# alibaba/euler

Measured on NVIDIA H100. Metric: sampled_edges_per_sec, higher is better.
Workload: dtype u64 ids / f32 weights+features (f64 CDF compare)

## Files before the change

euler_b200/csrc/internal.h:

```cpp
#pragma once
#include <cuda_runtime.h>
#include <stdint.h>

#include <string.h>

#include <atomic>
#include <string>
#include <type_traits>
#include <vector>

#include "../../include/euler_b200.h"
#include "common.cuh"

namespace eu {

void set_error(const char* fmt, ...);
extern std::atomic<uint64_t> g_launches;

#define EU_CUDA(call)                                                                    \
  do {                                                                                   \
    cudaError_t _e = (call);                                                             \
    if (_e != cudaSuccess) {                                                             \
      ::eu::set_error("%s:%d %s -> %s", __FILE__, __LINE__, #call, cudaGetErrorString(_e)); \
      return EU_ERR_CUDA;                                                                \
// ... 68 lines not shown
  float type_fwc_sum = 0.f;
  float* d_type_prob = nullptr;
  int32_t* d_type_alias = nullptr;
  std::vector<int64_t> sampler_order;
  std::vector<std::string> edge_type_names, node_type_names;
  std::vector<std::string> dense_feature_names;
  std::vector<std::string> sparse_feature_names, binary_feature_names;
  std::vector<uint64_t> u64_slot_max;
  eu::DevEdges e{};
  bool edges_set = false;
  struct EdgeSampler { int64_t n = 0; const int64_t* order = nullptr; const float* prob = nullptr; const int32_t* alias = nullptr; float fwc_sum = 0.f; };
  std::vector<EdgeSampler> edge_samplers;
  std::vector<std::string> edge_dense_names, edge_sparse_names, edge_binary_names;
  bool labels_built = false;
  std::vector<std::string> labels;
  int32_t* d_label_ptr = nullptr;
  unsigned long long* d_label_ids = nullptr;

  template <typename T>
  int alloc(T** p, int64_t count) {
    size_t bytes = (size_t)(count > 0 ? count : 1) * sizeof(T);
    bytes = (bytes + 255) & ~(size_t)255;
    void* q = nullptr;
    cudaError_t e = cudaMalloc(&q, bytes);
    if (e != cudaSuccess) {
      eu::set_error("cudaMalloc(%zu) -> %s", bytes, cudaGetErrorString(e));
      return EU_ERR_CUDA;
    }
    allocs.push_back(q);
    hbm_bytes += (int64_t)bytes;
    *p = (T*)q;
    return EU_OK;
  }
  template <typename T>
  int host_alloc(T** host, T** dev, int64_t count) {
    const size_t bytes = (size_t)(count > 0 ? count : 1) * sizeof(T);
    void* q = nullptr;
    cudaError_t e = cudaHostAlloc(&q, bytes, cudaHostAllocMapped);
    if (e != cudaSuccess) {
      cudaGetLastError();
      eu::set_error("cudaHostAlloc(%zu, mapped) -> %s", bytes, cudaGetErrorString(e));
      return EU_ERR_CUDA;
    }
    host_allocs.push_back(q);
    host_bytes += (int64_t)bytes;
    void* qd = nullptr;
    e = cudaHostGetDevicePointer(&qd, q, 0);
    if (e != cudaSuccess) { eu::set_error("cudaHostGetDevicePointer -> %s", cudaGetErrorString(e)); return EU_ERR_CUDA; }
    *host = (T*)q;
    *dev = (T*)qd;
    return EU_OK;
  }
};

struct EuRngState {
  uint32_t x;
  uint32_t x_prev;
  unsigned long long draws;
  unsigned long long calls;
  unsigned int blocks_done;
  unsigned int pad2;
  unsigned long long key;
};

struct eu_ctx {
  eu_graph* g = nullptr;
  eu_rng_kind rng = EU_RNG_MINSTD;
  uint64_t seed = 0;
  cudaStream_t stream = nullptr;
  EuRngState* d_rng = nullptr;
  int n_eng = 1;
  int64_t cap_rows = 0;
  eu::HashSlot* d_dedup = nullptr;
  int64_t tab_set_slots = 0;
  int32_t* d_first = nullptr;
  int64_t* d_rowof = nullptr;
  uint8_t* d_elig = nullptr;
  uint32_t* d_state = nullptr;
  uint32_t* d_emask = nullptr;
  uint32_t* d_woff = nullptr;
  uint32_t* d_blkpre = nullptr;
  uint32_t* d_blkmul = nullptr;
  int32_t* d_live = nullptr;
  int32_t* d_dup = nullptr;
  unsigned int* d_nlive = nullptr;
  unsigned long long* d_front[2] = {nullptr, nullptr};
  int64_t agg_rows = 0, agg_slots = 0;
  unsigned long long* d_agg_tab = nullptr;
  int32_t* d_agg_src = nullptr;
  int32_t* d_agg_rep = nullptr;
  uint32_t* d_agg_slot = nullptr;
  unsigned int* d_agg_nrep = nullptr;
  void* d_misc = nullptr;
  int64_t misc_bytes = 0;
  float* d_walkv = nullptr;
  long long walkv_cap = 0;
  cudaStream_t aux[2] = {nullptr, nullptr};
  cudaEvent_t ev_fork = nullptr, ev_join[2] = {nullptr, nullptr};
  void* h_pin = nullptr;
  int64_t pin_bytes = 0;
  void* d_stage = nullptr;
  int64_t stage_bytes = 0;
  bool prof = false;
  struct ProfRec { const char* name; int64_t rows; cudaEvent_t e0, e1; };
  std::vector<ProfRec> prof_recs;
};

struct EuProfScope {
  eu_ctx* c; size_t idx;
  EuProfScope(eu_ctx* c_, const char* name, int64_t rows) : c(c_), idx((size_t)-1) {
    if (!c->prof) return;
    eu_ctx::ProfRec r{name, rows, nullptr, nullptr};
    cudaEventCreate(&r.e0); cudaEventCreate(&r.e1);
    cudaEventRecord(r.e0, c->stream);
    c->prof_recs.push_back(r);
    idx = c->prof_recs.size() - 1;
  }
  ~EuProfScope() { if (idx != (size_t)-1) cudaEventRecord(c->prof_recs[idx].e1, c->stream); }
};

namespace eu {
static constexpr int64_t kRepeatMinRows = (int64_t)1 << 17;
int ctx_reserve(eu_ctx* c, int64_t rows, int64_t table_slots);
int64_t hop_scratch_rows(int nb, int64_t rows_b);
int64_t hop_table_slots(int nb, int64_t rows_b);
int64_t hop_table_cap(int64_t rows_b);
int ctx_misc(eu_ctx* c, int64_t bytes);
inline size_t a256(size_t b) { return (b + 255) & ~(size_t)255; }
struct EdgeOrder;
int segmented_row_sum(eu_ctx* c, const float* rows, const float* w, const EdgeOrder& o, const int32_t* row, int64_t E, int64_t n,
                      int dim, float* out);
size_t ragged_scan_bytes(int64_t M);
int sparse_entry_ptr(eu_ctx* c, const int64_t* nodes, int64_t M, int32_t fid, void* tmp, size_t tmp_bytes, int64_t* ptr);
int agg_reserve(eu_ctx* c, int64_t rows, int64_t table_slots);
int refuse_growth_in_capture(eu_ctx* c, const char* what);
int graph_build_sampler(eu_graph* g);
int feat_storage_check(const eu_feat_storage* in, int64_t n, const char* who, eu_feat_storage* st);
int graph_build_labels(eu_graph* g);
void graph_label_list(const std::vector<int64_t>& order, int64_t n, const int64_t* bin_ptr, const uint8_t* bin_val, int32_t S,
                      int32_t fid, std::vector<std::string>* labels, std::vector<int32_t>* row_label);
__global__ void k_advance_engine(EuRngState* rng, unsigned long long uniforms);
__global__ void k_ragged_stats(const long long* __restrict__ ptr, int64_t rows, long long* __restrict__ stats);
int agnn_dot(eu_ctx* c, const float* a, const float* b, const int32_t* ia, const int32_t* ib, int64_t E, int dim,
             const float* beta, float* dot, float* scaled);
int get_node_weight(eu_ctx* c, const int64_t* nodes, int64_t B, float* out);
int launch_state_scan(eu_ctx* c, int64_t rows, unsigned long long uniforms_per_row);
int hop(eu_ctx* c, const unsigned long long* seeds, int64_t rows, const int32_t* etypes, int32_t K,
        int32_t count, int64_t default_node, unsigned long long* eng_ids, int64_t* out_ids,
        float* out_w, int32_t* out_t, int hop_index, bool pre_inserted, bool insert_next, int nb,
        const int32_t* rows_act = nullptr, bool raw = false);
}
```

euler_b200/csrc/mp_ops.cu:

```cuda
#include <stdlib.h>

#include <cooperative_groups.h>

#include <algorithm>

#include "segment.cuh"

namespace cg = cooperative_groups;

namespace eu {

__device__ __forceinline__ float4 ldg4(const float* p) { return __ldg(reinterpret_cast<const float4*>(p)); }
__device__ __forceinline__ void st4(float* p, float4 v) { *reinterpret_cast<float4*>(p) = v; }

template <typename T, bool VEC, int P>
__global__ void __launch_bounds__(256) k_feature(DevGraph g, const unsigned long long* __restrict__ ids,
                                                 int64_t M, int32_t dim, int G, int32_t soff, int32_t sdim,
                                                 float* __restrict__ out) {
  const int sh = 31 - __clz(G);
  const int sub = (int)(threadIdx.x & (G - 1));
  const int64_t stride = ((int64_t)gridDim.x * blockDim.x) >> sh;
  for (int64_t i = (blockIdx.x * (int64_t)blockDim.x + threadIdx.x) >> sh; i < M; i += stride) {
    const int64_t row = sdim > 0 ? lookup_row(g, ids[i]) : -1;
    const int32_t fd = sdim;
    float* o = out + i * (int64_t)dim;
    const T* f = row >= 0 ? feat_row<T, P>(g, row) + soff : nullptr;
    if (VEC) {
      for (int32_t d = sub * 4; d < dim; d += G * 4) {
        float4 v = make_float4(0.f, 0.f, 0.f, 0.f);
        if (f && d < fd) v = feat_ld4(f + d);
        st4(o + d, v);
      }
    } else {
      for (int32_t d = sub; d < dim; d += G) o[d] = (f && d < fd) ? feat_ld(f + d) : 0.f;
    }
  }
}

template <bool VEC>
__global__ void __launch_bounds__(256) k_gather(const float* __restrict__ params, int64_t D,
                                                const int32_t* __restrict__ idx, int64_t E, int G,
                                                float* __restrict__ out) {
  const int64_t tid = blockIdx.x * (int64_t)blockDim.x + threadIdx.x;
  const int64_t i = tid >> (31 - __clz(G));
  const int sub = (int)(tid & (G - 1));
  if (i >= E) return;
  const float* src = params + (int64_t)__ldg(idx + i) * D;
  float* o = out + i * D;
  if (VEC) {
    for (int64_t d = sub * 4; d < D; d += G * 4) st4(o + d, ldg4(src + d));
  } else {
    for (int64_t d = sub; d < D; d += G) o[d] = __ldg(src + d);
  }
}

enum { OP_ADD = 0, OP_MAX = 1, OP_MEAN = 2 };

template <int OP, bool VEC>
__global__ void __launch_bounds__(256) k_scatter_sorted(const float* __restrict__ upd, int64_t D,
                                                        const int32_t* __restrict__ idx, int64_t E,
                                                        int64_t size, int G, const int* unsorted,
                                                        float* __restrict__ out) {
  if (*unsorted) return;
  const int64_t tid = blockIdx.x * (int64_t)blockDim.x + threadIdx.x;
  const int64_t r = tid >> (31 - __clz(G));
  const int sub = (int)(tid & (G - 1));
  if (r >= size) return;
  const int64_t b = key_lower_bound(idx, E, r), e = key_lower_bound(idx, E, r + 1);
  const float init = OP == OP_MAX ? -1e9f : 0.f;
  const float denom = __fadd_rn((float)(e - b), 1e-7f);
  float* o = out + r * D;
  if (VEC) {
    for (int64_t d = sub * 4; d < D; d += G * 4) {
      float4 acc = make_float4(init, init, init, init);
      for (int64_t k = b; k < e; ++k) {
        float4 v = ldg4(upd + k * D + d);
        if (OP == OP_MAX) {
          acc.x = v.x > acc.x ? v.x : acc.x; acc.y = v.y > acc.y ? v.y : acc.y;
          acc.z = v.z > acc.z ? v.z : acc.z; acc.w = v.w > acc.w ? v.w : acc.w;
        } else {
          acc.x = __fadd_rn(acc.x, v.x); acc.y = __fadd_rn(acc.y, v.y);
          acc.z = __fadd_rn(acc.z, v.z); acc.w = __fadd_rn(acc.w, v.w);
        }
      }
      if (OP == OP_MEAN) {
        acc.x = __fdiv_rn(acc.x, denom); acc.y = __fdiv_rn(acc.y, denom);
        acc.z = __fdiv_rn(acc.z, denom); acc.w = __fdiv_rn(acc.w, denom);
      }
      st4(o + d, acc);
    }
  } else {
    for (int64_t d = sub; d < D; d += G) {
      float acc = init;
      for (int64_t k = b; k < e; ++k) {
        float v = __ldg(upd + k * D + d);
        if (OP == OP_MAX) acc = v > acc ? v : acc; else acc = __fadd_rn(acc, v);
      }
      if (OP == OP_MEAN) acc = __fdiv_rn(acc, denom);
      o[d] = acc;
    }
  }
}

__global__ void k_fill_if(float* __restrict__ out, int64_t n, float v, const int* unsorted) {
  if (!*unsorted) return;
  int64_t i = blockIdx.x * (int64_t)blockDim.x + threadIdx.x;
  const int64_t stride = (int64_t)gridDim.x * blockDim.x;
  for (; i < n; i += stride) out[i] = v;
}

__device__ __forceinline__ void atomic_max_f32(float* addr, float v) {
  if (v != v) return;
  if (__float_as_int(v) >= 0) atomicMax(reinterpret_cast<int*>(addr), __float_as_int(v));
  else atomicMin(reinterpret_cast<unsigned int*>(addr), __float_as_uint(v));
}

template <int OP, bool VEC>
__global__ void __launch_bounds__(256) k_scatter_atomic(const float* __restrict__ upd, int64_t D,
                                                        const int32_t* __restrict__ idx, int64_t E, int G,
                                                        const int* unsorted, float* __restrict__ out,
                                                        float* __restrict__ cnt) {
  if (!*unsorted) return;
  const int64_t tid = blockIdx.x * (int64_t)blockDim.x + threadIdx.x;
  const int64_t i = tid >> (31 - __clz(G));
  const int sub = (int)(tid & (G - 1));
  if (i >= E) return;
  const int64_t r = __ldg(idx + i);
  float* o = out + r * D;
  const float* u = upd + i * D;
  if (OP == OP_MEAN && sub == 0) atomicAdd(cnt + r, 1.0f);
  if (VEC && OP != OP_MAX) {
    for (int64_t d = sub * 4; d < D; d += G * 4) atomicAdd(reinterpret_cast<float4*>(o + d), ldg4(u + d));
  } else {
    const int step = VEC ? 4 : 1;
    for (int64_t d = sub * step; d < D; d += G * step)
      for (int q = 0; q < step; ++q) {
        if (OP == OP_MAX) atomic_max_f32(o + d + q, __ldg(u + d + q));
        else atomicAdd(o + d + q, __ldg(u + d + q));
      }
  }
}

__global__ void k_mean_div(float* __restrict__ out, int64_t D, int64_t size, const float* __restrict__ cnt,
                           const int* unsorted) {
  if (!*unsorted) return;
  int64_t i = blockIdx.x * (int64_t)blockDim.x + threadIdx.x;
  if (i < size * D) out[i] = __fdiv_rn(out[i], __fadd_rn(cnt[i / D], 1e-7f));
}

__global__ void __launch_bounds__(256) k_sage_classify(DevGraph g, const unsigned long long* __restrict__ ids, int64_t rows,
                                                       int32_t count, unsigned long long* tab, unsigned long long mask,
                                                       int32_t* __restrict__ src, int32_t* __restrict__ reps,
                                                       uint32_t* __restrict__ rep_slot, unsigned int* n_rep) {
  const int64_t stride = (int64_t)gridDim.x * blockDim.x;
  for (int64_t r = blockIdx.x * (int64_t)blockDim.x + threadIdx.x; r < rows; r += stride) {
    const unsigned long long* seg = ids + r * count;
    unsigned long long h = 0;
    bool any = false;
#pragma unroll 4
    for (int32_t j = 0; j < count; ++j) {
      const unsigned long long id = __ldg(seg + j);
      any |= lookup_row(g, id) >= 0;
      h = mix64(h + id + 1);
    }
    if (!any) { src[r] = -1; continue; }
    const unsigned long long tag = h & 0xFFFFFFFF00000000ull;
    unsigned long long p = h & mask;
    while (true) {
      unsigned long long sl = *reinterpret_cast<volatile unsigned long long*>(tab + p);
      if (sl == 0ull) {
        sl = atomicCAS(tab + p, 0ull, tag | (unsigned long long)(r + 1));
        if (sl == 0ull) {
          src[r] = (int32_t)r;
          const cg::coalesced_group grp = cg::coalesced_threads();
          unsigned int q = 0;
          if (grp.thread_rank() == 0) q = atomicAdd(n_rep, grp.size());
          q = grp.shfl(q, 0) + grp.thread_rank();
          reps[q] = (int32_t)r;
          rep_slot[q] = (uint32_t)p;
          break;
        }
      }
      if ((sl & 0xFFFFFFFF00000000ull) == tag) {
        const int64_t o = (int64_t)(sl & 0xFFFFFFFFull) - 1;
        const unsigned long long* os = ids + o * count;
        bool same = true;
#pragma unroll 4
        for (int32_t j = 0; j < count; ++j) same &= __ldg(seg + j) == __ldg(os + j);
        if (same) { src[r] = (int32_t)o; break; }
      }
      p = (p + 1) & mask;
    }
  }
}

template <typename T, int NV, bool FULL, int P>
__global__ void __launch_bounds__(256) k_sage_mean(DevGraph g, const unsigned long long* __restrict__ ids,
                                                   int64_t rows, const int32_t* __restrict__ list, const unsigned int* __restrict__ n_list,
                                                   int32_t count, bool mean, float* __restrict__ out) {
  const int lane = threadIdx.x & 31;
  const int32_t fd = FULL ? NV * 128 : g.feat_dim;
  const int64_t nwarps = ((int64_t)gridDim.x * blockDim.x) >> 5;
  const int64_t n = list ? (int64_t)__ldg(n_list) : rows;
  for (int64_t q = (blockIdx.x * (int64_t)blockDim.x + threadIdx.x) >> 5; q < n; q += nwarps) {
  const int64_t r = list ? (int64_t)__ldg(list + q) : q;
  float4 acc[NV];
#pragma unroll
  for (int v = 0; v < NV; ++v) acc[v] = make_float4(0.f, 0.f, 0.f, 0.f);
  for (int32_t j0 = 0; j0 < count; j0 += 32) {
    int32_t my = -1;
    if (j0 + lane < count) my = (int32_t)lookup_row(g, __ldg(ids + r * count + j0 + lane));
    unsigned valid = __ballot_sync(0xffffffffu, my >= 0);
    while (valid) {
      float4 v[4][NV];
      int n = 0;
#pragma unroll
      for (int q = 0; q < 4; ++q) {
        if (valid) {
          const int j = __ffs(valid) - 1;
          valid &= valid - 1;
          const int32_t row = __shfl_sync(0xffffffffu, my, j);
          const T* p = feat_row<T, P>(g, row, fd, lane * 4);
#pragma unroll
          for (int t = 0; t < NV; ++t) v[q][t] = (FULL || lane * 4 + t * 128 < fd) ? feat_ld4(p + t * 128) : make_float4(0.f, 0.f, 0.f, 0.f);
          n = q + 1;
        }
      }
#pragma unroll
      for (int q = 0; q < 4; ++q) {
        if (q < n) {
#pragma unroll
          for (int t = 0; t < NV; ++t) {
            acc[t].x = __fadd_rn(acc[t].x, v[q][t].x); acc[t].y = __fadd_rn(acc[t].y, v[q][t].y);
            acc[t].z = __fadd_rn(acc[t].z, v[q][t].z); acc[t].w = __fadd_rn(acc[t].w, v[q][t].w);
          }
        }
      }
    }
  }
  const float denom = __fadd_rn((float)count, 1e-7f);
  float* o = out + r * (int64_t)fd + lane * 4;
#pragma unroll
  for (int t = 0; t < NV; ++t) {
    float4 a = acc[t];
    if (mean) { a.x = __fdiv_rn(a.x, denom); a.y = __fdiv_rn(a.y, denom); a.z = __fdiv_rn(a.z, denom); a.w = __fdiv_rn(a.w, denom); }
    if (FULL || lane * 4 + t * 128 < fd) st4(o + t * 128, a);
  }
  }
}

template <typename T, int P>
__global__ void __launch_bounds__(256) k_sage_mean_generic(DevGraph g, const unsigned long long* __restrict__ ids,
                                                           int64_t rows, const int32_t* __restrict__ list, const unsigned int* __restrict__ n_list,
                                                           int32_t count, int32_t dim, bool mean, float* __restrict__ out) {
  const int lane = threadIdx.x & 31;
  const int32_t fd = g.feat_dim;
  const float denom = __fadd_rn((float)count, 1e-7f);
  const int64_t nwarps = ((int64_t)gridDim.x * blockDim.x) >> 5;
  const int64_t n = list ? (int64_t)__ldg(n_list) : rows;
  for (int64_t q = (blockIdx.x * (int64_t)blockDim.x + threadIdx.x) >> 5; q < n; q += nwarps) {
    const int64_t r = list ? (int64_t)__ldg(list + q) : q;
    for (int32_t d = lane; d < dim; d += 32) {
      float acc = 0.f;
      for (int32_t j = 0; j < count; ++j) {
        const int64_t row = lookup_row(g, __ldg(ids + r * count + j));
        acc = __fadd_rn(acc, (row >= 0 && d < fd) ? feat_ld(feat_row<T, P>(g, row, fd, 0) + d) : 0.f);
      }
      out[r * (int64_t)dim + d] = mean ? __fdiv_rn(acc, denom) : acc;
    }
  }
}
// ... 72 lines not shown
}

template <typename T, int P>
static int launch_sage_mean(eu_ctx* c, const DevGraph& d, const unsigned long long* ids, int64_t rows, const int32_t* reps,
                            const unsigned int* nrep, int32_t count, int32_t dim, bool mean, bool v4, unsigned blocks, float* out) {
  cudaStream_t s = c->stream;
  if (v4 && dim == 128) k_sage_mean<T, 1, true, P><<<blocks, 256, 0, s>>>(d, ids, rows, reps, nrep, count, mean, out);
  else if (v4 && dim == 256) k_sage_mean<T, 2, true, P><<<blocks, 256, 0, s>>>(d, ids, rows, reps, nrep, count, mean, out);
  else if (v4 && dim <= 128) k_sage_mean<T, 1, false, P><<<blocks, 256, 0, s>>>(d, ids, rows, reps, nrep, count, mean, out);
  else if (v4 && dim <= 256) k_sage_mean<T, 2, false, P><<<blocks, 256, 0, s>>>(d, ids, rows, reps, nrep, count, mean, out);
  else if (v4 && dim <= 512) k_sage_mean<T, 4, false, P><<<blocks, 256, 0, s>>>(d, ids, rows, reps, nrep, count, mean, out);
  else if (v4) k_sage_mean<T, 8, false, P><<<blocks, 256, 0, s>>>(d, ids, rows, reps, nrep, count, mean, out);
  else k_sage_mean_generic<T, P><<<blocks, 256, 0, s>>>(d, ids, rows, reps, nrep, count, dim, mean, out);
  EU_LAUNCHED();
  return EU_OK;
}

}

using namespace eu;

extern "C" {

int eu_get_dense_feature(eu_ctx* c, const int64_t* nodes, int64_t M, int32_t fid, int32_t dim, float* out) {
  if (!c || M < 0 || dim < 0 || (M > 0 && (!nodes || (dim > 0 && !out)))) { set_error("eu_get_dense_feature: bad argument"); return EU_ERR_INVALID; }
  EU_CUDA(cudaSetDevice(c->g->device));
  if (M == 0 || dim == 0) return EU_OK;
  const DevGraph& d = c->g->d;
  int32_t soff, sdim;
  dense_slot(d, fid, &soff, &sdim);
  const bool vec = (dim % 4 == 0) && (d.feat_dim % 4 == 0) && (soff % 4 == 0) && (sdim % 4 == 0) && aligned16(out);
  const int G = vec ? group_lanes(dim / 4) : (dim >= 32 ? 32 : 1);
  const unsigned blocks = capped_grid(ceil_div(M * G, 256), "EU_FEATURE_CTAS", 0);
  EuProfScope ps(c, "k_feature", M);
  with_feat(d, [&](auto t, auto p) {
    using T = typename decltype(t)::type;
    constexpr int P = decltype(p)::value;
    auto k = vec ? k_feature<T, true, P> : k_feature<T, false, P>;
    k<<<blocks, 256, 0, c->stream>>>(d, (const unsigned long long*)nodes, M, dim, G, soff, sdim, out);
  });
  EU_LAUNCHED();
  return EU_OK;
}

int eu_gather(eu_ctx* c, const float* params, int64_t N, int64_t D, const int32_t* idx, int64_t E, float* out) {
  (void)N;
  if (!c || D <= 0 || E < 0 || (E > 0 && (!params || !idx || !out))) { set_error("eu_gather: bad argument"); return EU_ERR_INVALID; }
  EU_CUDA(cudaSetDevice(c->g->device));
  if (E == 0) return EU_OK;
  const bool vec = (D % 4 == 0) && aligned16(params) && aligned16(out);
  const int G = vec ? group_lanes(D / 4) : (D >= 32 ? 32 : 1);
  const unsigned blocks = (unsigned)ceil_div(E * G, 256);
  if (vec) k_gather<true><<<blocks, 256, 0, c->stream>>>(params, D, idx, E, G, out);
  else k_gather<false><<<blocks, 256, 0, c->stream>>>(params, D, idx, E, G, out);
  EU_LAUNCHED();
  return EU_OK;
}

int eu_scatter_add(eu_ctx* c, const float* u, int64_t D, const int32_t* idx, int64_t E, int64_t size, float* out) {
  return scatter<OP_ADD>(c, u, D, idx, E, size, out);
}
int eu_scatter_max(eu_ctx* c, const float* u, int64_t D, const int32_t* idx, int64_t E, int64_t size, float* out) {
  return scatter<OP_MAX>(c, u, D, idx, E, size, out);
}
int eu_scatter_mean(eu_ctx* c, const float* u, int64_t D, const int32_t* idx, int64_t E, int64_t size, float* out) {
  return scatter<OP_MEAN>(c, u, D, idx, E, size, out);
}

static int fanout_aggregate(eu_ctx* c, const int64_t* nbr_ids, int64_t rows, int32_t count, int32_t dim, bool mean, float* out) {
  if (!c || rows < 0 || count < 0 || dim <= 0 || (rows > 0 && (!nbr_ids || !out))) { set_error("eu_sage_mean_aggregate: bad argument"); return EU_ERR_INVALID; }
  EU_CUDA(cudaSetDevice(c->g->device));
  if (rows == 0) return EU_OK;
  cudaStream_t s = c->stream;
  const DevGraph& d = c->g->d;
  const unsigned long long* ids = (const unsigned long long*)nbr_ids;
  const bool dedup = rows >= kRepeatMinRows && rows < ((int64_t)1 << 31);
  int64_t cap = 64;
  while (cap < 2 * rows) cap <<= 1;
  if (dedup) {
    int rc = agg_reserve(c, rows, cap);
    if (rc) return rc;
    EU_CUDA(cudaMemsetAsync(c->d_agg_nrep, 0, sizeof(unsigned int), s));
    EuProfScope ps(c, "k_sage_classify", rows);
    k_sage_classify<<<capped_grid(ceil_div(rows, 256), "EU_SAGE_CTAS", 0), 256, 0, s>>>(d, ids, rows, count, c->d_agg_tab, (unsigned long long)cap - 1,
                                                                                      c->d_agg_src, c->d_agg_rep, c->d_agg_slot, c->d_agg_nrep);
    EU_LAUNCHED();
  }
  const unsigned blocks = capped_grid(ceil_div(rows * 32, 256), "EU_SAGE_CTAS", 0);
  const int32_t* reps = dedup ? c->d_agg_rep : nullptr;
  const unsigned int* nrep = c->d_agg_nrep;
  { EuProfScope ps(c, mean ? "k_sage_mean" : "k_sage_add", rows);
    const bool v4 = d.n < ((int64_t)1 << 31) && d.n_slots == 1 && dim == d.feat_dim && (dim & 3) == 0 && dim <= 1024 && aligned16(out) &&
                    aligned4_elems(d.feat, d.feat_dtype);
    const int rc = with_feat(d, [&](auto t, auto p) {
      return launch_sage_mean<typename decltype(t)::type, decltype(p)::value>(c, d, ids, rows, reps, nrep, count, dim, mean, v4, blocks, out);
    });
    if (rc) return rc; }
  if (!dedup) return EU_OK;
  { EuProfScope ps(c, "k_sage_broadcast", rows);
    const bool vec = (dim & 3) == 0 && aligned16(out);
    const int G = vec ? group_lanes(dim / 4) : (dim >= 32 ? 32 : 1);
    const unsigned bb = capped_grid(ceil_div(rows * G, 256), "EU_SAGE_CTAS", 0);
    if (vec) k_sage_broadcast<true><<<bb, 256, 0, s>>>(c->d_agg_src, rows, dim, G, c->d_agg_slot, nrep, c->d_agg_tab, out);
    else k_sage_broadcast<false><<<bb, 256, 0, s>>>(c->d_agg_src, rows, dim, G, c->d_agg_slot, nrep, c->d_agg_tab, out); }
  EU_LAUNCHED();
  return EU_OK;
}

int eu_sage_mean_aggregate(eu_ctx* c, const int64_t* nbr_ids, int64_t rows, int32_t count, int32_t dim, float* out) {
  return fanout_aggregate(c, nbr_ids, rows, count, dim, true, out);
}
int eu_sage_add_aggregate(eu_ctx* c, const int64_t* nbr_ids, int64_t rows, int32_t count, int32_t dim, float* out) {
  return fanout_aggregate(c, nbr_ids, rows, count, dim, false, out);
}

}
```

euler_b200/csrc/sample.cu:

```cuda
#include <algorithm>

#include <stdlib.h>

#include "internal.h"

namespace eu {

struct ETypes {
  int32_t K;
  int32_t v[EU_MAX_ETYPES];
};

struct Geom {
  int32_t nb;
  int32_t nblk_b;
  int64_t rows_b;
  int64_t rows_pad;
  int64_t cap_b;
  const int32_t* rows_act;
};

__global__ void k_dedup_insert(HashSlot* tabs, Geom gm, const unsigned long long* __restrict__ seeds) {
  const int b = blockIdx.y;
  const int64_t li = blockIdx.x * (int64_t)blockDim.x + threadIdx.x;
  const int64_t rows_here = gm.rows_act ? (int64_t)gm.rows_act[b] : gm.rows_b;
  if (li >= rows_here) return;
  const unsigned long long id = seeds[b * gm.rows_b + li];
  const unsigned act = __activemask();
  const unsigned peers = __match_any_sync(act, id);
  if ((threadIdx.x & 31) != __ffs(peers) - 1) return;
  dedup_insert_one(tabs + (int64_t)b * (gm.cap_b + 1), (unsigned long long)dedup_cap_eff(gm.cap_b, gm.rows_act, b) - 1, id, li);
}

__device__ __forceinline__ int64_t dedup_first(const HashSlot* tab, unsigned long long mask,
                                               unsigned long long id) {
  unsigned long long tag = id + 1;
  if (tag == 0ull) return (int64_t)tab[mask + 1].row;
  unsigned long long h = mix64(id) & mask;
  while (true) {
    const ulonglong2 s = *reinterpret_cast<const ulonglong2*>(tab + h);
    if (s.x == tag) return (int64_t)s.y;
    h = (h + 1) & mask;
  }
}

__device__ __forceinline__ float grp_cum_at(const DevGraph& g, int64_t row, int32_t t) {
  if (g.grp_cum) return __ldg(g.grp_cum + row * g.T + t);
  const int64_t b = g.grp_ptr[row], e = g.grp_ptr[row + 1];
  return e > b ? __ldg(g.cum_w + e - 1) : 0.f;
}

__device__ __forceinline__ bool row_eligible(const DevGraph& g, int64_t row, const ETypes& et, int mode) {
  if (row < 0) return false;
  const int32_t T = g.T;
  if (mode == 0) {
    int32_t t = et.v[0];
    if (t < 0 || t >= T) return false;
    return g.grp_ptr[row * T + t + 1] > g.grp_ptr[row * T + t];
  }
  if (mode == 1) {
    float s = 0.f;
    for (int32_t i = 0; i < et.K; ++i) {
      int32_t t = et.v[i];
      if (t < 0 || t >= T) return false;
      float pre = t > 0 ? grp_cum_at(g, row, t - 1) : 0.f;
      s = __fadd_rn(s, __fsub_rn(grp_cum_at(g, row, t), pre));
    }
    return s != 0.f;
  }
  return grp_cum_at(g, row, T - 1) != 0.f;
}

struct PrepOut {
  unsigned long long* eng_ids;
  long long* out_ids;
  float* out_w;
  int32_t* out_t;
  int32_t count;
  long long default_node;
  HashSlot* next_tabs;
  int64_t next_cap_b;
  int32_t* live;
  unsigned int* n_live;
  int32_t* dup;
  unsigned int* n_dup;
};

static constexpr int kPrepBlock = 256;

__global__ void __launch_bounds__(kPrepBlock) k_prepare(DevGraph g, const HashSlot* tabs, Geom gm,
                                                        const unsigned long long* __restrict__ seeds,
                                                        ETypes et, int mode, uint32_t F, unsigned long long draws_per_row,
                                                        int32_t* first, int64_t* rowof, uint32_t* emask, uint32_t* wmul,
                                                        uint32_t* blkpre, uint32_t* blkmul, EuRngState* rngs, PrepOut po) {
  __shared__ uint32_t s_w[kPrepBlock / 32];
  __shared__ uint32_t s_l[kPrepBlock / 32];
  __shared__ uint32_t s_d[kPrepBlock / 32];
  __shared__ uint32_t s_z[kPrepBlock / 32];
  __shared__ bool s_last;
  const int b = blockIdx.y;
  const int64_t li = blockIdx.x * (int64_t)kPrepBlock + threadIdx.x;
  const int64_t ii = b * gm.rows_pad + li;
  const int lane = threadIdx.x & 31, wid = threadIdx.x >> 5;
  EuRngState* rng = rngs + b;
  bool e = false;
  bool own = false;
  bool dflt = false;
  const int64_t rows_here = gm.rows_act ? (int64_t)gm.rows_act[b] : gm.rows_b;
  const uint32_t nblk_act = (uint32_t)max((int64_t)1, (rows_here + kPrepBlock - 1) / kPrepBlock);
  if (blockIdx.x >= nblk_act) return;
  if (li < rows_here) {
    const int64_t w = b * gm.rows_b + li;
    const unsigned long long id = seeds[w];
    const int64_t f = tabs ? dedup_first(tabs + (int64_t)b * (gm.cap_b + 1), (unsigned long long)dedup_cap_eff(gm.cap_b, gm.rows_act, b) - 1, id) : li;
    first[ii] = (int32_t)f;
    const int64_t row = lookup_row(g, id);
    own = row_eligible(g, row, et, mode);
    e = own && f == li;
    dflt = !own;
    if (own) rowof[ii] = row;
  }
  const uint32_t zm = __ballot_sync(0xffffffffu, dflt);
  if (zm) {
    const int64_t ob = (b * gm.rows_b + (li - lane)) * (int64_t)po.count;
    const uint32_t n = 32u * (uint32_t)po.count;
    for (uint32_t k = lane; k < n; k += 32) {
      if (!((zm >> (k / (uint32_t)po.count)) & 1u)) continue;
      if (po.eng_ids) po.eng_ids[ob + k] = 0ull;
      if (po.out_ids) { po.out_ids[ob + k] = po.default_node; po.out_w[ob + k] = 0.f; po.out_t[ob + k] = -1; }
    }
  }
  const uint32_t m = __ballot_sync(0xffffffffu, e);
  const uint32_t lm = po.dup ? m : __ballot_sync(0xffffffffu, own);
  const uint32_t dm = po.dup ? __ballot_sync(0xffffffffu, own && !e) : 0u;
  if (lane == 0) { s_w[wid] = __popc(m); s_l[wid] = __popc(lm); s_d[wid] = __popc(dm); s_z[wid] = zm; }
  __syncthreads();
  if (lane == 0) {
    uint32_t off = 0;
    for (int k = 0; k < wid; ++k) off += s_w[k];
    emask[ii >> 5] = m;
    uint32_t fp = 1, fb = F;
    for (; off; off >>= 1) { if (off & 1) fp = modmul(fp, fb); fb = modmul(fb, fb); }
    wmul[ii >> 5] = fp;
  }
  uint32_t* bp = blkpre + (int64_t)b * gm.nblk_b;
  if (threadIdx.x == 0) {
    uint32_t tot = 0, lt = 0, dt = 0;
    for (int k = 0; k < kPrepBlock / 32; ++k) {
      tot += s_w[k];
      const uint32_t l = s_l[k], d = s_d[k];
      s_l[k] = lt; s_d[k] = dt;
      lt += l; dt += d;
    }
    const uint32_t lbase = lt ? atomicAdd(po.n_live, lt) : 0u, dbase = dt ? atomicAdd(po.n_dup, dt) : 0u;
    for (int k = 0; k < kPrepBlock / 32; ++k) { s_l[k] += lbase; s_d[k] += dbase; }
    if (po.next_tabs)
      for (int k = 0; k < kPrepBlock / 32; ++k)
        if (s_z[k]) {
          const int64_t lz = blockIdx.x * (int64_t)kPrepBlock + k * 32 + (__ffs(s_z[k]) - 1);
          dedup_insert_one(po.next_tabs + (int64_t)b * (po.next_cap_b + 1), (unsigned long long)po.next_cap_b - 1, 0ull,
                           lz * (int64_t)po.count);
          break;
        }
    bp[blockIdx.x] = tot;
    __threadfence();
    s_last = atomicAdd(&rng->blocks_done, 1u) == nblk_act - 1;
  }
  __syncthreads();
  {
    const uint32_t below = (1u << lane) - 1u;
    if (e || (own && !po.dup)) po.live[s_l[wid] + __popc(lm & below)] = (int32_t)(b * gm.rows_b + li);
    else if (own) po.dup[s_d[wid] + __popc(dm & below)] = (int32_t)(b * gm.rows_b + li);
  }
  if (!s_last) return;
  __threadfence();
  __shared__ uint32_t s_scan[kPrepBlock];
  uint32_t carry = 0;
  for (uint32_t base = 0; base < nblk_act; base += kPrepBlock) {
    const uint32_t k = base + threadIdx.x;
    const uint32_t v = k < nblk_act ? __ldcg(bp + k) : 0u;
    s_scan[threadIdx.x] = v;
    __syncthreads();
    for (int off = 1; off < kPrepBlock; off <<= 1) {
      uint32_t t = threadIdx.x >= off ? s_scan[threadIdx.x - off] : 0u;
      __syncthreads();
      s_scan[threadIdx.x] += t;
      __syncthreads();
    }
    if (k < nblk_act) {
      uint32_t pre = carry + s_scan[threadIdx.x] - v;
      bp[k] = pre;
      uint32_t fp = 1, fb = F;
      for (; pre; pre >>= 1) { if (pre & 1) fp = modmul(fp, fb); fb = modmul(fb, fb); }
      blkmul[(int64_t)b * gm.nblk_b + k] = fp;
    }
    carry += s_scan[kPrepBlock - 1];
    __syncthreads();
  }
  if (threadIdx.x == 0) {
    uint32_t fp = 1, base = F;
    for (uint32_t t = carry; t; t >>= 1) { if (t & 1) fp = modmul(fp, base); base = modmul(base, base); }
    rng->x_prev = rng->x;
    rng->x = modmul(rng->x, fp);
    rng->draws += (unsigned long long)carry * draws_per_row;
    rng->blocks_done = 0;
  }
}

__global__ void __launch_bounds__(1024) k_state_scan(const uint8_t* __restrict__ elig, int64_t rows,
                                                     uint32_t F, unsigned long long draws_per_row,
                                                     uint32_t* state, EuRngState* rng) {
  __shared__ uint32_t s_part[1024];
  __shared__ uint32_t s_cnt[1024];
  const int t = threadIdx.x;
  const int64_t chunk = (rows + 1023) / 1024;
  const int64_t b = t * chunk, e = min(rows, b + chunk);
  uint32_t prod = 1, cnt = 0;
  for (int64_t i = b; i < e; ++i)
    if (elig[i]) { prod = modmul(prod, F); ++cnt; }
  s_part[t] = prod;
  s_cnt[t] = cnt;
  __syncthreads();
  for (int off = 1; off < 1024; off <<= 1) {
    uint32_t v = 1, c = 0;
    if (t >= off) { v = s_part[t - off]; c = s_cnt[t - off]; }
    __syncthreads();
    if (t >= off) { s_part[t] = modmul(s_part[t], v); s_cnt[t] += c; }
    __syncthreads();
  }
  const uint32_t x0 = rng->x;
  uint32_t run = modmul(x0, t > 0 ? s_part[t - 1] : 1u);
  for (int64_t i = b; i < e; ++i) {
    state[i] = run;
    if (elig[i]) run = modmul(run, F);
  }
  __syncthreads();
  if (t == 1023) {
    rng->x = modmul(x0, s_part[1023]);
    rng->draws += (unsigned long long)s_cnt[1023] * draws_per_row;
  }
}

struct SampleArgs {
  const unsigned long long* seeds;
  Geom gm;
  int32_t count;
  long long default_node;
  ETypes et;
  int mode;
  const int32_t* live;
  const unsigned int* n_live;
  const int32_t* first;
  const int64_t* rowof;
  const uint32_t* emask;
  const uint32_t* wmul;
// ... 191 lines not shown
      }
      int32_t etype = a.mode == 0 ? a.et.v[0] : 0;
      int64_t b = gb, e = ge;
      float lb = lim_b, le = lim_e;
      if (a.mode != 0) {
        const float tt = gt_threshold(pick_r(u_t, 0.f, tc_end));
        int k = lane_upper_bound(tc, 0, ntc - 1, tt, gmask, SG);
        etype = a.mode == 1 ? a.et.v[k] : k;
        b = gp[etype];
        e = gp[etype + 1] - 1;
        if (e < b) {
          bad = bad || active;
          b = base; e = base;
        }
        lb = b == base ? 0.f : __ldg(g.cum_w + b - 1);
        le = __ldg(g.cum_w + e);
      }
      const float thr = gt_threshold(pick_r(u_n, lb, le));
      int64_t m;
      float wgt;
      if (small_row) {
        int li2 = lane_upper_bound(c, (int)(b - base), (int)(e - base), thr, gmask, SG);
        float hi_v = __shfl_sync(gmask, c, li2, SG);
        float lo_v = __shfl_sync(gmask, c, li2 > 0 ? li2 - 1 : 0, SG);
        m = base + li2;
        wgt = __fsub_rn(hi_v, li2 > 0 ? lo_v : 0.f);
      } else if (mid_row) {
        int lo = (int)(b - base), hi = (int)(e - base);
        while (lo < hi) {
          const int mid = (lo + hi) >> 1;
          if (srow[mid] >= thr) hi = mid; else lo = mid + 1;
        }
        m = base + lo;
        wgt = __fsub_rn(srow[lo], lo > 0 ? srow[lo - 1] : 0.f);
      } else {
        m = b + bisect_clamped(g.cum_w + b, 0, (int32_t)(e - b), thr);
        float hi_v = __ldg(g.cum_w + m);
        float lo_v = m > base ? __ldg(g.cum_w + m - 1) : 0.f;
        wgt = __fsub_rn(hi_v, lo_v);
      }
      const unsigned long long nid = active ? __ldg(g.nbr + m) : 0ull;
      if (j0 == 0) {
        unsigned long long first_id = __shfl_sync(gmask, nid, 0, SG);
        keep = first_id != 0ull;
      }
      if (active) {
        if (a.eng_ids) a.eng_ids[obase + j] = nid;
        if (a.out_ids) {
          a.out_ids[obase + j] = keep ? (long long)nid : a.default_node;
          a.out_w[obase + j] = keep ? wgt : 0.f;
          a.out_t[obase + j] = keep ? etype : -1;
        }
      }
      if (!PHILOX && ntab && a.mode == 0) {
        const unsigned act = __ballot_sync(gmask, active);
        if (active) {
          const unsigned peers = __match_any_sync(act, nid);
          if (lane == __ffs(peers) - 1) dedup_insert_one(ntab, nmask, nid, nbase + j);
        }
      }
    }
    if (__any_sync(gmask, bad)) {
      for (int32_t j = sl; j < count; j += SG) {
        if (a.eng_ids) a.eng_ids[obase + j] = 0ull;
        if (a.out_ids) { a.out_ids[obase + j] = a.default_node; a.out_w[obase + j] = 0.f; a.out_t[obase + j] = -1; }
      }
    }
    if (!PHILOX && ntab && a.mode != 0) {
      for (int32_t j0 = 0; j0 < count; j0 += SG) {
        const int32_t j = j0 + sl;
        const bool active = j < count;
        const unsigned long long nid = active ? a.eng_ids[obase + j] : 0ull;
        const unsigned act = __ballot_sync(gmask, active);
        if (active) {
          const unsigned peers = __match_any_sync(act, nid);
          if (lane == __ffs(peers) - 1) dedup_insert_one(ntab, nmask, nid, nbase + j);
        }
      }
    }
    if (mid_row) __syncwarp(gmask);
  }
}

__global__ void __launch_bounds__(256) k_copy_dups(Geom gm, int32_t count, int sg_log, const int32_t* __restrict__ dup,
                                                   const unsigned int* __restrict__ n_dup, const int32_t* __restrict__ first,
                                                   unsigned long long* eng_ids, long long* out_ids, float* out_w, int32_t* out_t) {
  const int sl = threadIdx.x & ((1 << sg_log) - 1);
  const int64_t total = (int64_t)__ldg(n_dup);
  const int64_t stride = ((int64_t)gridDim.x * blockDim.x) >> sg_log;
  for (int64_t q = (blockIdx.x * (int64_t)blockDim.x + threadIdx.x) >> sg_log; q < total; q += stride) {
    const int64_t w = __ldg(dup + q);
    const int bidx = (int)(w / gm.rows_b);
    const int64_t li = w - bidx * gm.rows_b;
    const int64_t f = __ldg(first + bidx * gm.rows_pad + li);
    const int64_t src = (bidx * gm.rows_b + f) * count, dst = w * (int64_t)count;
    for (int32_t j = sl; j < count; j += 1 << sg_log) {
      if (eng_ids) eng_ids[dst + j] = eng_ids[src + j];
      if (out_ids) { out_ids[dst + j] = out_ids[src + j]; out_w[dst + j] = out_w[src + j]; out_t[dst + j] = out_t[src + j]; }
    }
  }
}

__global__ void k_bump_calls(EuRngState* rngs, int nb) {
  if (threadIdx.x < nb) rngs[threadIdx.x].calls += 1;
}

struct NodeSamplerDev {
  int32_t n_types;
  const unsigned long long* ids[EU_MAX_ETYPES];
  const float* prob[EU_MAX_ETYPES];
  const int32_t* alias[EU_MAX_ETYPES];
  long long n[EU_MAX_ETYPES];
  const float* type_prob;
  const int32_t* type_alias;
  int mode;
  int32_t type0;
  int32_t n_sub;
  int32_t sub_ids[EU_MAX_ETYPES];
  float sub_cum[EU_MAX_ETYPES];
};

__device__ __forceinline__ long long alias_next(const float* prob, const int32_t* alias, long long n,
                                                double u1, double u2) {
  long long col = (long long)floor(__dmul_rn((double)n, u1));
  bool coin = u2 < (double)__ldg(prob + col);
  return coin ? col : (long long)__ldg(alias + col);
}

template <bool PHILOX>
__global__ void k_sample_node(NodeSamplerDev s, int32_t count, int32_t upd, unsigned long long key,
                              EuRngState* rng, long long* out) {
  const int32_t j = blockIdx.x * blockDim.x + threadIdx.x;
  if (j < count) {
    double u[4] = {0, 0, 0, 0};
    if (PHILOX) {
      philox_uniform2(0x5A4D504C45ull, (uint32_t)j, (uint32_t)rng->calls, key, u[0], u[1]);
      philox_uniform2(0x5A4D504C46ull, (uint32_t)j, (uint32_t)rng->calls, key, u[2], u[3]);
      if (s.mode == 0) { u[2] = u[0]; u[3] = u[1]; }
    } else {
      uint32_t x = modmul(rng->x, modpow_a(2ull * upd * (unsigned long long)j));
      if (s.mode == 1) { u[0] = minstd_uniform(x); u[1] = minstd_uniform(x); }
      if (s.mode == 2) { u[0] = minstd_uniform(x); }
      u[2] = minstd_uniform(x);
      u[3] = minstd_uniform(x);
    }
    int32_t t = s.type0;
    if (s.mode == 1) {
      t = (int32_t)alias_next(s.type_prob, s.type_alias, s.n_types, u[0], u[1]);
    } else if (s.mode == 2) {
      double r = pick_r(u[0], 0.f, s.sub_cum[s.n_sub - 1]);
      int k = 0;
      while (k < s.n_sub - 1 && !((double)s.sub_cum[k] > r)) ++k;
      t = s.sub_ids[k];
    }
    long long col = alias_next(s.prob[t], s.alias[t], s.n[t], u[2], u[3]);
    out[j] = (long long)__ldg(s.ids[t] + col);
  }
}

__device__ __forceinline__ void advance_engine(EuRngState* rng, unsigned long long uniforms) {
  rng->x = modmul(rng->x, modpow_a(2ull * uniforms));
  rng->draws += uniforms;
  rng->calls += 1;
}

__global__ void k_advance_engine(EuRngState* rng, unsigned long long uniforms) { advance_engine(rng, uniforms); }

enum : unsigned { kTypeAbsent = 1u, kTypeRange = 2u, kTypeEmpty = 4u };

__global__ void k_check_types(const int32_t* __restrict__ types, int64_t n, int32_t n_types, unsigned int empty_types,
                              unsigned int* flag) {
  unsigned bad = 0;
  for (int64_t i = blockIdx.x * (int64_t)blockDim.x + threadIdx.x; i < n; i += (int64_t)gridDim.x * blockDim.x) {
    const int32_t t = __ldg(types + i);
    if (t == INT32_MIN) bad |= kTypeAbsent;
    else if (t < 0 || t >= n_types) bad |= kTypeRange;
    else if ((empty_types >> t) & 1u) bad |= kTypeEmpty;
  }
  bad = __reduce_or_sync(0xffffffffu, bad);
// ... 78 lines not shown
        int32_t K, int32_t count, int64_t default_node, unsigned long long* eng_ids,
        int64_t* out_ids, float* out_w, int32_t* out_t, int hop_index, bool pre_inserted, bool insert_next, int nb,
        const int32_t* rows_act, bool raw) {
  const int64_t rows = rows_b * nb;
  if (rows == 0 || count == 0) return EU_OK;
  if (nb < 1 || nb > c->n_eng) { set_error("hop: %d batches but the ctx has %d engines", nb, c->n_eng); return EU_ERR_INVALID; }
  const DevGraph& d = c->g->d;
  SampleArgs a{};
  int rc = classify(d, etypes, K, &a.et, &a.mode);
  if (rc) return rc;
  if (a.mode != 0 && d.T > 32) { set_error("T > 32 unsupported"); return EU_ERR_UNSUPPORTED; }
  cudaStream_t s = c->stream;
  Geom gm = make_geom(nb, rows_b);
  gm.rows_act = rows_act;
  a.seeds = seeds; a.gm = gm; a.count = count; a.default_node = default_node;
  a.eng_ids = eng_ids; a.out_ids = (long long*)out_ids; a.out_w = out_w; a.out_t = out_t;
  a.rngs = c->d_rng;
  {
    int need = std::min<int>(count, 32);
    if (a.mode == 1) need = std::max<int>(need, std::min<int>(a.et.K, 32));
    if (a.mode == 2) need = std::max<int>(need, std::min<int>(d.T, 32));
    a.sg_log = 0;
    while ((1 << a.sg_log) < need) ++a.sg_log;
  }
  static const int stage_rows = [] { const char* e = getenv("EU_SAMPLE_STAGE"); return e ? (atoi(e) != 0 ? 1 : 0) : 1; }();
  a.stage = stage_rows;
  static const int grid_ctas = [] { const char* e = getenv("EU_SAMPLE_CTAS"); return e ? std::min(8, std::max(1, atoi(e))) : 8; }();
  const int ctas = grid_ctas <= 5 ? 5 : grid_ctas == 6 ? 6 : 8;
  const unsigned blocks = (unsigned)std::min<int64_t>(ceil_div(ceil_div(rows * 32, (int64_t)(32 >> a.sg_log)), 256), kSMs * grid_ctas);
  if (c->rng == EU_RNG_PHILOX) {
    a.key = c->seed;
    { EuProfScope ps(c, "k_sample<philox>", rows); if (ctas == 6) k_sample<true, 6><<<blocks, 256, 0, s>>>(d, a); else k_sample<true, 8><<<blocks, 256, 0, s>>>(d, a); }
    EU_LAUNCHED();
    k_bump_calls<<<1, 64, 0, s>>>(c->d_rng, nb);
    EU_LAUNCHED();
    return EU_OK;
  }
  if (rows >= ((int64_t)1 << 31) || nb > 64) { set_error("rows >= 2^31 or more than 64 batches"); return EU_ERR_UNSUPPORTED; }
  const Geom ng = make_geom(nb, rows_b * count);
  const bool chain = insert_next && eng_ids;
  rc = ctx_reserve(c, std::max(gm.rows_pad, chain ? ng.rows_pad : 0) * nb, (std::max(gm.cap_b, chain ? ng.cap_b : 0) + 1) * nb);
  if (rc) return rc;
  const int tb = kPrepBlock;
  HashSlot* tabs = c->d_dedup + (hop_index & 1) * c->tab_set_slots;
  HashSlot* ntabs = c->d_dedup + ((hop_index + 1) & 1) * c->tab_set_slots;
  if (raw && (pre_inserted || insert_next)) { set_error("hop: raw mode does not chain"); return EU_ERR_INVALID; }
  if (!pre_inserted && !raw) {
    EuProfScope ps(c, "k_dedup_insert", rows);
    k_dedup_insert<<<dim3((unsigned)ceil_div(gm.rows_b, tb), (unsigned)nb), tb, 0, s>>>(tabs, gm, seeds);
    EU_LAUNCHED();
  }
  const unsigned long long upr = (unsigned long long)count * (a.mode == 0 ? 1 : 2);
  const uint32_t F = modpow_a(2ull * upr);
  { EuProfScope ps(c, "k_prepare", rows);
    PrepOut po{};
    po.eng_ids = eng_ids; po.out_ids = (long long*)out_ids; po.out_w = out_w; po.out_t = out_t;
    po.count = count; po.default_node = default_node;
    if (chain) { po.next_tabs = ntabs; po.next_cap_b = ng.cap_b; }
    po.live = c->d_live; po.n_live = c->d_nlive;
    if (!raw && rows >= kRepeatMinRows) { po.dup = c->d_dup; po.n_dup = c->d_nlive + 1; }
    EU_CUDA(cudaMemsetAsync(c->d_nlive, 0, 2 * sizeof(unsigned int), s));
    k_prepare<<<dim3((unsigned)gm.nblk_b, (unsigned)nb), tb, 0, s>>>(d, raw ? nullptr : tabs, gm, seeds, a.et, a.mode, F, upr, c->d_first,
                                                                     c->d_rowof, c->d_emask, c->d_woff, c->d_blkpre, c->d_blkmul,
                                                                     c->d_rng, po); }
  EU_LAUNCHED();
  a.first = c->d_first; a.rowof = c->d_rowof; a.emask = c->d_emask; a.wmul = c->d_woff; a.blkmul = c->d_blkmul;
  a.live = c->d_live; a.n_live = c->d_nlive;
  a.F = F;
  const uint32_t upd = a.mode == 0 ? 1u : 2u;
  for (uint32_t k = 0; k < 32; ++k) a.lanepow[k] = modpow_a(2ull * upd * k);
  a.stride = modpow_a(2ull * upd * (unsigned long long)(1u << a.sg_log));
  a.clear_tab = tabs;
  a.clear_n = raw ? 0 : (gm.cap_b + 1) * nb;
  if (chain) {
    a.next_tabs = ntabs;
    a.next_cap_b = ng.cap_b;
  }
  { EuProfScope ps(c, "k_sample<minstd>", rows);
    if (ctas == 5) k_sample<false, 5><<<blocks, 256, 0, s>>>(d, a);
    else if (ctas == 6) k_sample<false, 6><<<blocks, 256, 0, s>>>(d, a);
    else k_sample<false, 8><<<blocks, 256, 0, s>>>(d, a); }
  EU_LAUNCHED();
  if (!raw && rows >= kRepeatMinRows) {
    EuProfScope ps(c, "k_copy_dups", rows);
    k_copy_dups<<<blocks, 256, 0, s>>>(gm, count, a.sg_log, c->d_dup, c->d_nlive + 1, c->d_first, eng_ids, (long long*)out_ids, out_w, out_t);
    EU_LAUNCHED();
  }
  return EU_OK;
}

}

using namespace eu;

extern "C" {

int eu_sample_neighbor(eu_ctx* c, const int64_t* nodes, int64_t B, const int32_t* etypes, int32_t K,
                       int32_t count, int64_t default_node, int64_t* out_ids, float* out_w,
                       int32_t* out_t) {
  if (!c || B < 0 || count < 0 || (K > 0 && !etypes)) { set_error("eu_sample_neighbor: bad argument"); return EU_ERR_INVALID; }
  EU_CUDA(cudaSetDevice(c->g->device));
  return hop(c, (const unsigned long long*)nodes, B, etypes, K, count, default_node, nullptr, out_ids, out_w, out_t, 0, false, false, 1);
}

int eu_sample_neighbor_raw(eu_ctx* c, const int64_t* nodes, int64_t B, const int32_t* etypes, int32_t K,
                           int32_t count, int64_t* out_ids, float* out_w, int32_t* out_t) {
  if (!c || B < 0 || count < 0 || (K > 0 && !etypes)) { set_error("eu_sample_neighbor_raw: bad argument"); return EU_ERR_INVALID; }
  EU_CUDA(cudaSetDevice(c->g->device));
  if (c->rng != EU_RNG_MINSTD) { set_error("eu_sample_neighbor_raw: exact-RNG contexts only (philox rows are keyed on the node id: duplicates would repeat)"); return EU_ERR_UNSUPPORTED; }
  return hop(c, (const unsigned long long*)nodes, B, etypes, K, count, 0, nullptr, out_ids, out_w, out_t, 0, false, false, 1,
             nullptr, true);
}

int eu_sample_fanout_batched(eu_ctx* c, const int64_t* nodes, int32_t nb, int64_t B, const int32_t* etypes, int32_t K,
                             const int32_t* counts, int32_t L, int64_t default_node, int64_t* const* out_ids,
                             float* const* out_w, int32_t* const* out_t) {
  if (!c || nb < 1 || B < 0 || L < 0 || !counts || (K > 0 && !etypes)) { set_error("eu_sample_fanout: bad argument"); return EU_ERR_INVALID; }
  EU_CUDA(cudaSetDevice(c->g->device));
  if (nb > c->n_eng) { set_error("eu_sample_fanout_batched: %d batches but the ctx has %d engines (eu_ctx_set_engines)", nb, c->n_eng); return EU_ERR_INVALID; }
  for (int l = 0; l < L; ++l)
    if (counts[l] < 0) { set_error("negative count"); return EU_ERR_INVALID; }
  for (int l = 0; l < L; ++l)
    if (counts[l] == 0) { L = l; break; }
  if (B == 0) return EU_OK;
  int64_t rows_b = B, max_rows = hop_scratch_rows(nb, B), max_slots = hop_table_slots(nb, B), widest = B * nb;
  for (int l = 0; l < L; ++l) {
    rows_b *= counts[l];
    if (l + 1 < L) { max_rows = std::max(max_rows, hop_scratch_rows(nb, rows_b)); max_slots = std::max(max_slots, hop_table_slots(nb, rows_b)); }
    widest = std::max(widest, rows_b * nb);
  }
  int rc = ctx_reserve(c, std::max(max_rows, widest), max_slots);
  if (rc) return rc;
  const unsigned long long* seeds = (const unsigned long long*)nodes;
  rows_b = B;
  for (int l = 0; l < L; ++l) {
    unsigned long long* eng = (l + 1 < L) ? c->d_front[l & 1] : nullptr;
    rc = hop(c, seeds, rows_b, etypes + (int64_t)l * K, K, counts[l], default_node, eng,
             out_ids ? out_ids[l] : nullptr, out_w ? out_w[l] : nullptr, out_t ? out_t[l] : nullptr,
             l, l > 0 && c->rng == EU_RNG_MINSTD, l + 1 < L, nb);
    if (rc) return rc;
    seeds = eng;
    rows_b *= counts[l];
  }
  return EU_OK;
}

int eu_sample_fanout(eu_ctx* c, const int64_t* nodes, int64_t B, const int32_t* etypes, int32_t K,
                     const int32_t* counts, int32_t L, int64_t default_node, int64_t* const* out_ids,
                     float* const* out_w, int32_t* const* out_t) {
  return eu_sample_fanout_batched(c, nodes, 1, B, etypes, K, counts, L, default_node, out_ids, out_w, out_t);
}

int eu_sample_fanout_with_feature(eu_ctx* c, const int64_t* nodes, int64_t B, const int32_t* etypes, int32_t K, const int32_t* counts,
                                  int32_t L, int64_t default_node, int64_t* const* out_ids, float* const* out_w, int32_t* const* out_t,
                                  int64_t* const* eng_ids, int32_t n_dense, const int32_t* dense_fids, const int32_t* dense_dims,
                                  float* const* out_dense, int32_t n_sparse, const int32_t* sparse_fids, int64_t* const* sparse_ptr,
                                  int64_t* sparse_total, int64_t* sparse_max_len) {
  const char* who = "eu_sample_fanout_with_feature";
  if (!c || B < 0 || L < 0 || (L > 0 && (!counts || !out_ids || !out_w || !out_t || !eng_ids)) || (K > 0 && !etypes) || n_dense < 0 ||
      n_sparse < 0 || (n_dense > 0 && (!dense_fids || !dense_dims || !out_dense)) ||
      (n_sparse > 0 && (!sparse_fids || !sparse_ptr || !sparse_total || !sparse_max_len))) {
    set_error("%s: bad argument", who);
    return EU_ERR_INVALID;
  }
  for (int l = 0; l < L; ++l)
    if (counts[l] < 1) { set_error("%s: counts must be positive", who); return EU_ERR_INVALID; }
  EU_CUDA(cudaSetDevice(c->g->device));
  std::vector<int64_t> rows(L + 1, B);
// ... 138 lines not shown
```

Measured before the change: 6.012 billion.

## Stage classify ids through shared memory and store dup source pairs

k_sage_classify now has each warp cooperatively copy its 32 rows' neighbor ids into padded shared memory with async copies, so hashing and the equality check read coalesced staged data instead of strided per-thread global loads. The dup list now stores (dest, source) int2 pairs written by the prep kernel. This lets k_copy_dups skip the division and the extra lookup in the first array, and its grid is resized to groups of up to 256 threads per row. Costs are more shared memory and a changed dup buffer layout, and the classify grid is no longer capped by the env override.

```diff
diff --git a/euler_b200/csrc/internal.h b/euler_b200/csrc/internal.h
--- a/euler_b200/csrc/internal.h
+++ b/euler_b200/csrc/internal.h
@@ -174,7 +174,7 @@
   uint32_t* d_blkpre = nullptr;
   uint32_t* d_blkmul = nullptr;
   int32_t* d_live = nullptr;
-  int32_t* d_dup = nullptr;
+  int2* d_dup = nullptr;
   unsigned int* d_nlive = nullptr;
   unsigned long long* d_front[2] = {nullptr, nullptr};
   int64_t agg_rows = 0, agg_slots = 0;
diff --git a/euler_b200/csrc/mp_ops.cu b/euler_b200/csrc/mp_ops.cu
--- a/euler_b200/csrc/mp_ops.cu
+++ b/euler_b200/csrc/mp_ops.cu
@@ -1,3 +1,4 @@
+#include <cuda_pipeline_primitives.h>
 #include <stdlib.h>
 
 #include <cooperative_groups.h>
@@ -148,21 +149,49 @@
   if (i < size * D) out[i] = __fdiv_rn(out[i], __fadd_rn(cnt[i / D], 1e-7f));
 }
 
-__global__ void __launch_bounds__(256) k_sage_classify(DevGraph g, const unsigned long long* __restrict__ ids, int64_t rows,
+static constexpr int kClsChunk = 16;
+static constexpr int kClsStride = kClsChunk + 1;
+
+__global__ void __launch_bounds__(256, 4) k_sage_classify(DevGraph g, const unsigned long long* __restrict__ ids, int64_t rows,
                                                        int32_t count, unsigned long long* tab, unsigned long long mask,
                                                        int32_t* __restrict__ src, int32_t* __restrict__ reps,
                                                        uint32_t* __restrict__ rep_slot, unsigned int* n_rep) {
-  const int64_t stride = (int64_t)gridDim.x * blockDim.x;
-  for (int64_t r = blockIdx.x * (int64_t)blockDim.x + threadIdx.x; r < rows; r += stride) {
+  __shared__ unsigned long long s_ids[256 / 32][32 * kClsStride];
+  const int lane = threadIdx.x & 31;
+  unsigned long long* st = s_ids[threadIdx.x >> 5];
+  const int64_t nwarps = ((int64_t)gridDim.x * blockDim.x) >> 5;
+  const bool whole = count <= kClsChunk;
+  for (int64_t r0 = ((blockIdx.x * (int64_t)blockDim.x + threadIdx.x) >> 5) * 32; r0 < rows; r0 += nwarps * 32) {
+    const int nr = rows - r0 < 32 ? (int)(rows - r0) : 32;
+    const int64_t r = r0 + lane;
     const unsigned long long* seg = ids + r * count;
     unsigned long long h = 0;
     bool any = false;
-#pragma unroll 4
-    for (int32_t j = 0; j < count; ++j) {
-      const unsigned long long id = __ldg(seg + j);
-      any |= lookup_row(g, id) >= 0;
-      h = mix64(h + id + 1);
-    }
+    for (int32_t j0 = 0; j0 < count; j0 += kClsChunk) {
+      const int w = min(count - j0, kClsChunk);
+      const int n = nr * w;
+      const int i0 = lane / w, t0 = lane - i0 * w, di = 32 / w, dt = 32 - di * w;
+      const unsigned long long* p = ids + (r0 + i0) * count + j0 + t0;
+      const int64_t dp = (int64_t)di * count + dt, pwrap = count - w;
+      int s = i0 * kClsStride + t0, t = t0;
+      const int ds = di * kClsStride + dt, swrap = kClsStride - w;
+      __syncwarp();
+      for (int e = lane; e < n; e += 32) {
+        __pipeline_memcpy_async(st + s, p, sizeof(unsigned long long));
+        p += dp; s += ds; t += dt;
+        if (t >= w) { t -= w; p += pwrap; s += swrap; }
+      }
+      __pipeline_commit();
+      __pipeline_wait_prior(0);
+      __syncwarp();
+      if (lane < nr)
+        for (int u = 0; u < w; ++u) {
+          const unsigned long long id = st[lane * kClsStride + u];
+          any |= lookup_row(g, id) >= 0;
+          h = mix64(h + id + 1);
+        }
+    }
+    if (lane >= nr) continue;
     if (!any) { src[r] = -1; continue; }
     const unsigned long long tag = h & 0xFFFFFFFF00000000ull;
     unsigned long long p = h & mask;
@@ -186,7 +215,7 @@
         const unsigned long long* os = ids + o * count;
         bool same = true;
 #pragma unroll 4
-        for (int32_t j = 0; j < count; ++j) same &= __ldg(seg + j) == __ldg(os + j);
+        for (int32_t j = 0; j < count; ++j) same &= (whole ? st[lane * kClsStride + j] : __ldg(seg + j)) == __ldg(os + j);
         if (same) { src[r] = (int32_t)o; break; }
       }
       p = (p + 1) & mask;
@@ -425,8 +454,8 @@
     if (rc) return rc;
     EU_CUDA(cudaMemsetAsync(c->d_agg_nrep, 0, sizeof(unsigned int), s));
     EuProfScope ps(c, "k_sage_classify", rows);
-    k_sage_classify<<<capped_grid(ceil_div(rows, 256), "EU_SAGE_CTAS", 0), 256, 0, s>>>(d, ids, rows, count, c->d_agg_tab, (unsigned long long)cap - 1,
-                                                                                      c->d_agg_src, c->d_agg_rep, c->d_agg_slot, c->d_agg_nrep);
+    k_sage_classify<<<(unsigned)ceil_div(rows, 256), 256, 0, s>>>(d, ids, rows, count, c->d_agg_tab, (unsigned long long)cap - 1,
+                                                                  c->d_agg_src, c->d_agg_rep, c->d_agg_slot, c->d_agg_nrep);
     EU_LAUNCHED();
   }
   const unsigned blocks = capped_grid(ceil_div(rows * 32, 256), "EU_SAGE_CTAS", 0);
diff --git a/euler_b200/csrc/sample.cu b/euler_b200/csrc/sample.cu
--- a/euler_b200/csrc/sample.cu
+++ b/euler_b200/csrc/sample.cu
@@ -82,7 +82,7 @@
   int64_t next_cap_b;
   int32_t* live;
   unsigned int* n_live;
-  int32_t* dup;
+  int2* dup;
   unsigned int* n_dup;
 };
 
@@ -106,13 +106,14 @@
   bool e = false;
   bool own = false;
   bool dflt = false;
+  int64_t f = li;
   const int64_t rows_here = gm.rows_act ? (int64_t)gm.rows_act[b] : gm.rows_b;
   const uint32_t nblk_act = (uint32_t)max((int64_t)1, (rows_here + kPrepBlock - 1) / kPrepBlock);
   if (blockIdx.x >= nblk_act) return;
   if (li < rows_here) {
     const int64_t w = b * gm.rows_b + li;
     const unsigned long long id = seeds[w];
-    const int64_t f = tabs ? dedup_first(tabs + (int64_t)b * (gm.cap_b + 1), (unsigned long long)dedup_cap_eff(gm.cap_b, gm.rows_act, b) - 1, id) : li;
+    f = tabs ? dedup_first(tabs + (int64_t)b * (gm.cap_b + 1), (unsigned long long)dedup_cap_eff(gm.cap_b, gm.rows_act, b) - 1, id) : li;
     first[ii] = (int32_t)f;
     const int64_t row = lookup_row(g, id);
     own = row_eligible(g, row, et, mode);
@@ -170,7 +171,7 @@
   {
     const uint32_t below = (1u << lane) - 1u;
     if (e || (own && !po.dup)) po.live[s_l[wid] + __popc(lm & below)] = (int32_t)(b * gm.rows_b + li);
-    else if (own) po.dup[s_d[wid] + __popc(dm & below)] = (int32_t)(b * gm.rows_b + li);
+    else if (own) po.dup[s_d[wid] + __popc(dm & below)] = make_int2((int32_t)(b * gm.rows_b + li), (int32_t)(b * gm.rows_b + f));
   }
   if (!s_last) return;
   __threadfence();
@@ -528,19 +529,24 @@
   }
 }
 
-__global__ void __launch_bounds__(256) k_copy_dups(Geom gm, int32_t count, int sg_log, const int32_t* __restrict__ dup,
-                                                   const unsigned int* __restrict__ n_dup, const int32_t* __restrict__ first,
-                                                   unsigned long long* eng_ids, long long* out_ids, float* out_w, int32_t* out_t) {
-  const int sl = threadIdx.x & ((1 << sg_log) - 1);
+static constexpr int kCopyThreads = 256;
+
+__global__ void __launch_bounds__(kCopyThreads) k_copy_dups(int32_t count, const int2* __restrict__ dup,
+                                                            const unsigned int* __restrict__ n_dup,
+                                                            unsigned long long* eng_ids, long long* out_ids, float* out_w,
+                                                            int32_t* out_t) {
+  const int span = min(count, kCopyThreads);
+  const int per_cta = kCopyThreads / span;
+  const int sub = threadIdx.x / span;
+  if (sub >= per_cta) return;
+  const int j0 = threadIdx.x - sub * span;
   const int64_t total = (int64_t)__ldg(n_dup);
-  const int64_t stride = ((int64_t)gridDim.x * blockDim.x) >> sg_log;
-  for (int64_t q = (blockIdx.x * (int64_t)blockDim.x + threadIdx.x) >> sg_log; q < total; q += stride) {
-    const int64_t w = __ldg(dup + q);
-    const int bidx = (int)(w / gm.rows_b);
-    const int64_t li = w - bidx * gm.rows_b;
-    const int64_t f = __ldg(first + bidx * gm.rows_pad + li);
-    const int64_t src = (bidx * gm.rows_b + f) * count, dst = w * (int64_t)count;
-    for (int32_t j = sl; j < count; j += 1 << sg_log) {
+  const int64_t stride = (int64_t)gridDim.x * per_cta;
+  for (int64_t q = blockIdx.x * (int64_t)per_cta + sub; q < total; q += stride) {
+    const int2 wf = __ldg(dup + q);
+    const int64_t src = (int64_t)wf.y * count, dst = (int64_t)wf.x * count;
+#pragma unroll 1
+    for (int32_t j = j0; j < count; j += span) {
       if (eng_ids) eng_ids[dst + j] = eng_ids[src + j];
       if (out_ids) { out_ids[dst + j] = out_ids[src + j]; out_w[dst + j] = out_w[src + j]; out_t[dst + j] = out_t[src + j]; }
     }
@@ -785,8 +791,10 @@
     else k_sample<false, 8><<<blocks, 256, 0, s>>>(d, a); }
   EU_LAUNCHED();
   if (!raw && rows >= kRepeatMinRows) {
+    const int64_t per_cta = kCopyThreads / std::min<int32_t>(count, kCopyThreads);
+    const unsigned cblocks = (unsigned)std::min<int64_t>(ceil_div(rows, per_cta), kSMs * (2048 / kCopyThreads));
     EuProfScope ps(c, "k_copy_dups", rows);
-    k_copy_dups<<<blocks, 256, 0, s>>>(gm, count, a.sg_log, c->d_dup, c->d_nlive + 1, c->d_first, eng_ids, (long long*)out_ids, out_w, out_t);
+    k_copy_dups<<<cblocks, kCopyThreads, 0, s>>>(count, c->d_dup, c->d_nlive + 1, eng_ids, (long long*)out_ids, out_w, out_t);
     EU_LAUNCHED();
   }
   return EU_OK;
```

New measurement: 6.016 billion (median of 6 runs). No clear change (+0.1%).
